# SludgePhD/Compeg

Measured on AMD Instinct MI355X. Metric: Mpixels/s decoded (4K 4:2:2 restart-interval baseline JPEG -> RGBA8 in HBM), higher is better.
Workload: dtype u32 bit-reader / i16 levels / f32 IDCT / u8 RGBA

## Files before the change

compeg_amd/csrc/desc.cpp:

```cpp
#include <cstdlib>
#include <cstring>
#include <vector>

#include "device_types.h"
#include "front.h"
#include "kernels_body.h"
#include "coop_body.h"

namespace compeg {

void fill_desc(const ImageData &img, ImageDesc &d);
void fill_coop(const ImageData &img, ImageDesc &d);
uint32_t max_wave_span(const uint32_t *starts, size_t nstarts, size_t nwords, uint32_t intervals, uint32_t group);
bool walk_state_shared(const ImageDesc &a, const ImageDesc &b);

void fill_desc(const ImageData &img, ImageDesc &d)
{
    d.walk = nullptr;
    const Metadata &md = img.metadata;
    memset(&d, 0, sizeof d);
    d.l2_entries = uint32_t(img.l2.size());
    d.fast_off = uint32_t((img.l2.size() + 1) & ~size_t(1));
    d.standard_entropy = (img.flags & COMPEG_PARSE_STANDARD_ENTROPY) ? 1u : 0u;
    d.total_intervals = md.total_restart_intervals;
    d.restart_interval = md.restart_interval;
    d.dus_per_mcu = md.dus_per_mcu;
    d.width_mcus = md.width_mcus;
    d.mcu_w = md.max_hsample * 8;
    d.mcu_h = md.max_vsample * 8;
    d.total_dus = img.total_dus();
    uint32_t k = 0;
    for (uint32_t c = 0; c < 3; c++) {
        const Component &cm = md.components[c];
        d.du_base[c] = k;
        for (uint32_t i = 0; i < cm.hsample * cm.vsample && k < kMaxDusPerMcu; i++, k++)
            d.comp_of_du |= c << (2 * k);
        d.dc_table[c] = cm.dchuff < 4 ? cm.dchuff : 4;
        d.ac_table[c] = cm.achuff < 4 ? cm.achuff : 4;
        d.fast_table[c] = (cm.achuff == 1 || cm.achuff == 3) ? cm.achuff >> 1 : 2;
        d.dc_quant[c] = md.qtables[cm.qtable & 3][0];
        d.hsample[c] = cm.hsample;
        d.vsample[c] = cm.vsample;
        for (int z = 0; z < kRetained; z++)
            d.quant[c][z] = float(md.qtables[cm.qtable & 3][z]);
        d.dc_fast_table[c] = (cm.dchuff == 0 || cm.dchuff == 2) ? cm.dchuff >> 1 : 2;
    }
    fill_coop(img, d);
    d.total_mcus = img.total_mcus();
    const bool is422 = md.dus_per_mcu == 4 && md.components[0].hsample == 2 && md.components[0].vsample == 1 &&
                       md.components[1].hsample == 1 && md.components[1].vsample == 1 &&
                       md.components[2].hsample == 1 && md.components[2].vsample == 1;
    bool ok = is422 && md.restart_interval != 0 && md.restart_interval <= (1u << 18) && d.zero_du_ok != 0;
    if (ok) {
        const uint32_t pair0 = (d.dc_fast_table[0] & 1u) | ((d.fast_table[0] & 1u) << 1);
        uint32_t pair1 = pair0;
        for (uint32_t c = 1; c < 3; c++) {
            const uint32_t pr = (d.dc_fast_table[c] & 1u) | ((d.fast_table[c] & 1u) << 1);
            if (pr != pair0 && pair1 == pair0)
                pair1 = pr;
            ok = ok && (pr == pair0 || pr == pair1);
        }
    }
    for (uint32_t c = 0; c < 3 && ok; c++) {
        ok = d.fast_table[c] < 2 && d.dc_fast_table[c] < 2;
        const uint16_t *l1 = img.l1 + size_t(d.dc_table[c] & 3u) * 256;
        for (uint32_t i = 0; i < 256 && ok; i++) {
            const uint16_t e = l1[i];
            if (!(e & 0x8000u)) {
                ok = (e & 0xffu) <= 15u;
                continue;
            }
            for (uint32_t j = 0; j < 256 && ok; j++) {
                const size_t idx = size_t(e & 0x7fffu) + j;
                ok = idx >= img.l2.size() || (img.l2[idx] & 0xffu) <= 15u;
            }
        }
    }
    d.mcu_ok = ok ? 1u : 0u;
}

void fill_coop(const ImageData &img, ImageDesc &d)
{
    const Metadata &md = img.metadata;
    d.coop_ok = 0;
    d.zero_du_ok = 0;
    memset(d.zero_du, 0, sizeof d.zero_du);
    const bool is422 = md.dus_per_mcu == 4 && md.components[0].hsample == 2 && md.components[0].vsample == 1 &&
                       md.components[1].hsample == 1 && md.components[1].vsample == 1 &&
                       md.components[2].hsample == 1 && md.components[2].vsample == 1;
    if (!is422 || md.restart_interval == 0)
        return;
    for (uint32_t c = 0; c < 3; c++)
        if (d.fast_table[c] >= 2 || d.dc_fast_table[c] >= 2)
            return;
    std::vector<uint16_t> l1(kL1Entries, 0);
    memcpy(l1.data(), img.l1, sizeof img.l1);
    const uint32_t none[4] = {0, 0, 0, 0};
    ImageDesc t = d;
    t.l2 = img.l2.data();
    t.words = nullptr;
    t.nwords = 0;
    HuffShared s{};
    s.l1 = l1.data();
    s.l2 = img.l2.empty() ? l1.data() : img.l2.data();
    s.l2_staged = uint32_t(img.l2.size());
    s.win = none;
    s.win_base = 0;
    s.win_len = 4;
    for (uint32_t c = 0; c < 3; c++) {
        PrefetchReader r;
        r.buf = 0;
        r.left = 0x80000000u;
        r.next_word = 0;
        r.pre = 0;
        ImageDesc tq = t;
        tq.standard_entropy = 0;
        const int32_t diff = decode_dc_diff(r, tq, s, d.dc_table[c] * 256u);
        if (diff < -32767 || diff > 32767)
            return;
        int16_t slot[kDuSlotBytes / 2] = {0};
        decode_ac_loop<false>(r, tq, s, d.ac_table[c] * 256u, slot);
        d.zero_du[c][0] = int16_t(diff);
        for (int z = 1; z < kRetained; z++)
            d.zero_du[c][z] = slot[z];
    }
    d.zero_du_ok = 1;
    d.coop_ok = md.restart_interval <= kCoopMaxRestart ? 1u : 0u;
}

bool walk_state_shared(const ImageDesc &a, const ImageDesc &b)
// ... 25 lines not shown
```

compeg_amd/csrc/device_types.h:

```cpp
#pragma once

#include <cstdint>

namespace compeg {

constexpr int kWave = 64;
constexpr int kRetained = 32;
constexpr int kMaxDusPerMcu = 6;
constexpr uint32_t kStripMcus = 32;

constexpr uint32_t kFastBits = 11;
constexpr uint32_t kFastEntries = 1u << kFastBits;
constexpr uint32_t kFastAdvEob = 64;
constexpr uint32_t kFastEscape = 15u;

constexpr uint32_t fast_entry(uint32_t ref, uint32_t zrl_advance)
{
    return (((ref & 0xffu) == 0u ? kFastAdvEob : ((ref & 0xffu) == 0xf0u ? zrl_advance : ((ref >> 4) & 15u) + 1u)) << 9) |
           ((((ref >> 8) & 31u) + (ref & 15u)) << 4) | (ref & 15u);
}

constexpr uint32_t kDcFastBits = 9;
constexpr uint32_t kDcFastEntries = 1u << kDcFastBits;

#ifndef CG_COOP_LEAN_MAX
#define CG_COOP_LEAN_MAX 40
#endif
constexpr uint32_t kCoopLeanMaxRestart = CG_COOP_LEAN_MAX;
struct CoopShape {
    uint32_t dpi, ipw, rounds, lpi, count, list_cap;
};
constexpr uint32_t kCoopSlotListCap = 20;
constexpr CoopShape coop_shape(uint32_t restart_interval, uint32_t waves)
{
    CoopShape sh{};
    sh.dpi = 4u * restart_interval;
    const uint32_t room = uint32_t(kWave) * (waves ? waves : 1u);
    sh.ipw = (sh.dpi != 0u && sh.dpi <= room) ? room / sh.dpi : 1u;
    sh.rounds = (sh.ipw * sh.dpi + uint32_t(kWave) - 1u) / uint32_t(kWave);
    const uint32_t share = (sh.dpi + (waves ? waves : 1u) - 1u) / (waves ? waves : 1u);
    const uint32_t fit = uint32_t(kWave) / sh.ipw;
    sh.lpi = share < fit ? (share ? share : 1u) : fit;
    sh.count = 1u + (sh.lpi - 1u) / 4u;
    const uint32_t per_sub = (sh.dpi + sh.count - 1u) / sh.count;
    sh.list_cap = (restart_interval > kCoopLeanMaxRestart && per_sub > 10u) ? ((per_sub + 15u) & ~3u) : kCoopSlotListCap;
    return sh;
}

constexpr int kDuSlotBytes = 80;

struct alignas(16) McuState {
    uint32_t info;
    int32_t pred[3];
};
constexpr uint32_t kMcuDead = 1u << 11;

struct ImageDesc {
    const uint32_t *words;
    const uint32_t *starts;
    const uint16_t *l1;
    const uint16_t *l2;
    uint32_t nwords;
    uint32_t nstarts;
    uint32_t l2_entries;
    uint32_t fast_off;
    uint32_t fast_table[3];
    uint32_t standard_entropy;
    uint32_t dc_fast_table[3];
    uint32_t coop_ok;
    uint32_t zero_du_ok;
    int16_t zero_du[3][kRetained];
    const uint32_t *walk;
    uint32_t total_intervals;
    uint32_t restart_interval;
    uint32_t dus_per_mcu;
    uint32_t width_mcus;
    uint32_t mcu_w, mcu_h;
    uint32_t total_dus;
    uint32_t comp_of_du;
    uint32_t dc_table[3];
    uint32_t ac_table[3];
    uint32_t dc_quant[3];
    uint32_t hsample[3], vsample[3];
    uint32_t du_base[3];
    float quant[3][kRetained];
    int16_t *ac;
    int32_t *dc;
    uint8_t *out;
    uint32_t out_w, out_h;
    uint32_t out_alloc_h;
    uint32_t out_pitch;
    uint32_t first_huff_block;
    uint32_t first_idct_block;
    uint32_t *mcu_word;
    McuState *mcu_state;
    uint32_t mcu_ok;
    uint32_t total_mcus;
};

struct HuffLdsPlan {
    uint32_t l2_entries_in_lds;
    uint32_t window_words;
    uint32_t waves_per_block;
    uint32_t total_bytes;
    uint32_t waves_that_fit;
    bool window_cut;
};

}
```

compeg_amd/csrc/kernels.hip:

```cpp
#include <hip/hip_runtime.h>

#include <algorithm>
#include <atomic>
#include <cstdio>
#include <cstdlib>

#include "kernels_body.h"
#include "coop_body.h"
#include "walk_body.h"
#include "kernels.h"
#include "lab.h"

namespace compeg {

struct DeviceLimits {
    uint32_t cus, lds_bytes;
};
static DeviceLimits device_limits()
{
    static std::atomic<uint64_t> known[64];
    int dev = 0;
    const bool indexed = hipGetDevice(&dev) == hipSuccess && dev >= 0 && dev < 64;
    if (indexed) {
        const uint64_t k = known[dev].load(std::memory_order_relaxed);
// ... 85 lines not shown
    if (wave_first >= d.total_intervals)
        return;

    HuffShared s;
    s.l1 = l1;
    s.l2 = l2;
    s.l2_staged = umin(l2_in_lds, d.fast_off + 2u * kFastEntries);
    s.win = win;
    s.win_base = win_base;
    s.win_len = win_len;
    s.du_slots = reinterpret_cast<uint8_t *>(win) + align16(window_words * 4u);
    entropy_wave_to_records<SAMPLES>(d, s, wave_first + lane, lane);
}

__global__ void __launch_bounds__(1024)
entropy_kernel(const ImageDesc *__restrict__ descs, uint32_t l2_in_lds, uint32_t window_words)
{
    entropy_kernel_body<false>(descs, l2_in_lds, window_words);
}

__global__ void __launch_bounds__(768)
entropy_samples_kernel(const ImageDesc *__restrict__ descs, uint32_t l2_in_lds, uint32_t window_words)
{
    entropy_kernel_body<true>(descs, l2_in_lds, window_words);
}

struct WindowAhead {
    const ImageDesc *descs;
    uint32_t image;
    bool any;
    uint32_t first;
    uint32_t window_words, lane;
    uint32_t *win;
    uint32_t raw_base, raw_end, base, len, sink;
    uint32_t *queue;
    uint32_t next, drawn, stride, units, waves_per_image, group;

    __device__ __forceinline__ void at(uint32_t du, uint32_t du_total)
    {
        if (queue) {
            if (du == 0u && lane == 0u)
                drawn = atomicAdd(queue, 1u);
            if (du == 1u) {
                next = (stride + uint32_t(__builtin_amdgcn_readfirstlane(int(drawn)))) * group;
                any = next < units;
                if (any) {
                    image = uint32_t(__builtin_amdgcn_readfirstlane(int(next / waves_per_image)));
                    first = uint32_t(__builtin_amdgcn_readfirstlane(int((next % waves_per_image) * kWave)));
                }
            }
        }
        if (!any)
            return;
        const ImageDesc *dn = descs + image;
        if (du == (queue ? 1u : 0u))
            wave_window_fetch(*dn, first, raw_base, raw_end);
        if (du_total >= 8u && du == (du_total >= 10u ? du_total - 8u : 2u)) {
            uint32_t b, l;
            wave_window_from(*dn, raw_base, raw_end, window_words, b, l);
            const uint32_t have = dn->nwords > b ? umin(l, dn->nwords - b) : 0u;
            auto *words = CG_GLOBAL(const uint32_t, dn->words);
            for (uint32_t v = lane * 32u; v < have; v += kWave * 32u)
                sink ^= words[b + v];
        }
        if (du_total >= 8u && du == (du_total >= 10u ? du_total - 5u : 5u))
            asm volatile("" ::"v"(sink));
    }

    __device__ __forceinline__ void decoded(uint32_t du, uint32_t du_total)
    {
        if (!any || du + 1u != du_total)
            return;
        const ImageDesc *dn = descs + image;
        uint32_t b, l;
        wave_window_from(*dn, raw_base, raw_end, window_words, b, l);
        base = uint32_t(__builtin_amdgcn_readfirstlane(int(b)));
        len = uint32_t(__builtin_amdgcn_readfirstlane(int(l)));
        stage_window(*dn, win, base, len, lane);
        __builtin_amdgcn_fence(__ATOMIC_RELEASE, "wavefront");
        __builtin_amdgcn_wave_barrier();
    }
};

template <class LAYOUT, uint32_t GROUP>
__device__ __forceinline__ void fused_kernel_body(const ImageDesc *__restrict__ descs, uint32_t l2_in_lds, uint32_t window_words,
                                                  uint32_t waves_per_image, uint32_t images, uint32_t *queue)
{
    constexpr uint32_t group = GROUP;
    extern __shared__ __attribute__((aligned(16))) uint8_t smem[];
    const uint32_t wave = uint32_t(__builtin_amdgcn_readfirstlane(int(threadIdx.x / kWave))), lane = threadIdx.x % kWave;
    uint32_t image = blockIdx.y, wave_first = (blockIdx.x * (blockDim.x / kWave) + wave) * kWave;
    bool has_work = true;
    if (waves_per_image) {
        const uint32_t flat = (blockIdx.x * (blockDim.x / kWave) + wave) * (queue ? group : 1u);
        image = flat / waves_per_image;
        wave_first = (flat % waves_per_image) * kWave;
        has_work = image < images;
        image = has_work ? image : images - 1u;
    }
    image = uint32_t(__builtin_amdgcn_readfirstlane(int(image)));
    wave_first = uint32_t(__builtin_amdgcn_readfirstlane(int(wave_first)));
    if (!waves_per_image && blockIdx.x * blockDim.x >= descs[image].total_intervals)
        return;
    has_work = has_work && wave_first < descs[image].total_intervals;

    uint16_t *l1 = reinterpret_cast<uint16_t *>(smem);
    uint16_t *l2 = l1 + kL1Entries;
    const uint32_t wave_area = align16(window_words * 4u) + kWave * kDuSlotBytes;
    uint8_t *wave_base = smem + align16((kL1Entries + l2_in_lds) * 2u);
    uint32_t *win = reinterpret_cast<uint32_t *>(wave_base + wave * wave_area);
    uint8_t *slots = reinterpret_cast<uint8_t *>(win) + align16(window_words * 4u);

    uint32_t win_base = 0, win_len = 0;
    if (has_work)
        wave_window(descs[image], wave_first, window_words, win_base, win_len);
    stage_luts_and_window(descs[image], l1, l2, l2_in_lds, threadIdx.x, blockDim.x, win, win_base, win_len, lane);
    __syncthreads();

    if (!has_work)
        return;

    const uint32_t stride = gridDim.x * (blockDim.x / kWave), units = waves_per_image * images;
    const uint32_t per_draw = waves_per_image && queue ? group : 1u;
    uint32_t flat = (blockIdx.x * (blockDim.x / kWave) + wave) * per_draw;
    for (;;) {
        const ImageDesc &d = descs[image];
        HuffShared s;
        s.l1 = l1;
        s.l2 = l2;
        s.l2_staged = umin(l2_in_lds, d.fast_off + 2u * kFastEntries);
        s.win = win;
        s.win_base = win_base;
        s.win_len = win_len;
        s.du_slots = slots;
        const bool draw = waves_per_image && queue && flat % per_draw == per_draw - 1u;
        flat += waves_per_image && queue ? 1u : stride;
        WindowAhead ahead;
        ahead.descs = descs;
        ahead.queue = draw ? queue : nullptr;
        ahead.stride = stride;
        ahead.units = units;
        ahead.waves_per_image = waves_per_image;
        ahead.group = per_draw;
        ahead.next = ahead.drawn = 0u;
        ahead.any = waves_per_image && !draw && flat < units;
        ahead.image = ahead.first = 0u;
        if (ahead.any) {
            ahead.image = uint32_t(__builtin_amdgcn_readfirstlane(int(flat / waves_per_image)));
            ahead.first = uint32_t(__builtin_amdgcn_readfirstlane(int((flat % waves_per_image) * kWave)));
        }
        ahead.window_words = window_words;
        ahead.lane = lane;
        ahead.win = win;
        ahead.sink = 0u;
        LAYOUT::decode(d, s, wave_first + lane, lane, ahead);
        if (!ahead.any)
            break;
        if (draw)
            flat = ahead.next;
        image = ahead.image;
        wave_first = ahead.first;
        win_base = ahead.base;
        win_len = ahead.len;
    }
}

constexpr uint32_t kMcuQueueGroup = 4;

template <bool WIDE, bool RECORDS = false>
struct Wave422 {
    template <class AHEAD>
    static __device__ __forceinline__ void decode(const ImageDesc &d, const HuffShared &s, uint32_t interval, uint32_t lane, AHEAD &ahead)
    {
        decode_wave_fused_422<AHEAD, WIDE, RECORDS>(d, s, interval, lane, ahead);
    }
};
#if !defined(CG_FUSED_BOUNDS) || !defined(COMPEG_LAB)
#define CG_FUSED_BOUNDS 768
#endif
__global__ void __launch_bounds__(CG_FUSED_BOUNDS)
decode_fused_422_kernel(const ImageDesc *__restrict__ descs, uint32_t l2_in_lds, uint32_t window_words,
                        uint32_t waves_per_image, uint32_t images, uint32_t *queue)
{
    fused_kernel_body<Wave422<false>, 1>(descs, l2_in_lds, window_words, waves_per_image, images, queue);
}
__global__ void __launch_bounds__(768)
decode_fused_422_mcu_kernel(const ImageDesc *__restrict__ descs, uint32_t l2_in_lds, uint32_t window_words,
                            uint32_t waves_per_image, uint32_t images, uint32_t *queue)
{
    fused_kernel_body<Wave422<true>, kMcuQueueGroup>(descs, l2_in_lds, window_words, waves_per_image, images, queue);
}
__global__ void __launch_bounds__(768)
decode_fused_422_mcu_rec_kernel(const ImageDesc *__restrict__ descs, uint32_t l2_in_lds, uint32_t window_words,
                                uint32_t waves_per_image, uint32_t images, uint32_t *queue)
{
    fused_kernel_body<Wave422<true, true>, kMcuQueueGroup>(descs, l2_in_lds, window_words, waves_per_image, images, queue);
}
template <int HS, int VS, int MC>
__device__ __forceinline__ void fused_layout_kernel_body(const ImageDesc *__restrict__ descs, uint32_t l2_in_lds, uint32_t window_words)
{
    extern __shared__ __attribute__((aligned(16))) uint8_t smem[];
    const ImageDesc &d = descs[blockIdx.y];
    const uint32_t first_interval = blockIdx.x * blockDim.x;
    if (first_interval >= d.total_intervals)
        return;
    uint16_t *l1 = reinterpret_cast<uint16_t *>(smem);
    uint16_t *l2 = l1 + kL1Entries;
    const uint32_t wave_area = align16(window_words * 4u) + kWave * kDuSlotBytes;
    uint8_t *wave_base = smem + align16((kL1Entries + l2_in_lds) * 2u);
    const uint32_t wave = uint32_t(__builtin_amdgcn_readfirstlane(int(threadIdx.x / kWave))), lane = threadIdx.x % kWave;
    uint32_t *win = reinterpret_cast<uint32_t *>(wave_base + wave * wave_area);
    const uint32_t wave_first = first_interval + wave * kWave;
    uint32_t win_base = 0, win_len = 0;
    if (wave_first < d.total_intervals)
        wave_window(d, wave_first, window_words, win_base, win_len);
    stage_luts_and_window(d, l1, l2, l2_in_lds, threadIdx.x, blockDim.x, win, win_base, win_len, lane);
    __syncthreads();
    if (wave_first >= d.total_intervals)
        return;
    HuffShared s;
    s.l1 = l1;
    s.l2 = l2;
    s.l2_staged = umin(l2_in_lds, d.fast_off + 2u * kFastEntries);
    s.win = win;
    s.win_base = win_base;
    s.win_len = win_len;
    s.du_slots = reinterpret_cast<uint8_t *>(win) + align16(window_words * 4u);
    decode_wave_fused_layout<HS, VS, MC>(d, s, wave_first + lane, lane);
}

__global__ void __launch_bounds__(512)
decode_fused_444_kernel(const ImageDesc *__restrict__ descs, uint32_t l2_in_lds, uint32_t window_words)
{
    fused_layout_kernel_body<1, 1, 2>(descs, l2_in_lds, window_words);
}
__global__ void __launch_bounds__(768)
decode_fused_444_single_kernel(const ImageDesc *__restrict__ descs, uint32_t l2_in_lds, uint32_t window_words)
{
    fused_layout_kernel_body<1, 1, 1>(descs, l2_in_lds, window_words);
}
__global__ void __launch_bounds__(512)
decode_fused_440_kernel(const ImageDesc *__restrict__ descs, uint32_t l2_in_lds, uint32_t window_words)
{
    fused_layout_kernel_body<1, 2, 2>(descs, l2_in_lds, window_words);
}
__global__ void __launch_bounds__(768)
decode_fused_440_single_kernel(const ImageDesc *__restrict__ descs, uint32_t l2_in_lds, uint32_t window_words)
{
    fused_layout_kernel_body<1, 2, 1>(descs, l2_in_lds, window_words);
}
__global__ void __launch_bounds__(512)
decode_fused_420_kernel(const ImageDesc *__restrict__ descs, uint32_t l2_in_lds, uint32_t window_words)
{
    fused_layout_kernel_body<2, 2, 1>(descs, l2_in_lds, window_words);
}

template <class WAVE>
__device__ __forceinline__ void fused_stream_kernel_body(const ImageDesc *__restrict__ descs, uint32_t l2_in_lds, uint32_t rows,
                                                         uint32_t stage_after, uint32_t stage_below, uint32_t waves_per_image, uint32_t images,
                                                         uint32_t *queue)
{
    extern __shared__ __attribute__((aligned(16))) uint8_t smem[];
    const uint32_t wave = uint32_t(__builtin_amdgcn_readfirstlane(int(threadIdx.x / kWave))), lane = threadIdx.x % kWave;
    uint32_t image = blockIdx.y, wave_first = (blockIdx.x * (blockDim.x / kWave) + wave) * kWave;
    bool has_work = true;
    if (waves_per_image) {
        const uint32_t flat = blockIdx.x * (blockDim.x / kWave) + wave;
// ... 981 lines not shown
```

compeg_amd/csrc/kernels_body.h:

```cpp
#pragma once

#include <cstdint>
#include <cstring>

#include "device_types.h"

#if defined(__HIPCC__)
#define CG_DEV __device__ __forceinline__
#else
#define CG_DEV static inline
#endif

#if defined(__HIP_DEVICE_COMPILE__)
#define CG_GLOBAL(T, p) (reinterpret_cast<__attribute__((address_space(1))) T *>(reinterpret_cast<uintptr_t>(p)))
#define CG_PIN_SCALAR(x) asm volatile("" : "+s"(x))
#else
#define CG_GLOBAL(T, p) (p)
#define CG_PIN_SCALAR(x) (void)(x)
#endif

#ifndef CG_IDCT_PACKED
#define CG_IDCT_PACKED 1
#endif
#ifndef CG_PRIO_IDCT
// ... 679 lines not shown
            uint32_t e2 = s.l2[idx < s.l2_staged ? idx : 0u];
            if (idx >= s.l2_staged)
                e2 = CG_GLOBAL(const uint16_t, d.l2)[idx < d.l2_entries ? idx : 0u];
            e = idx < d.l2_entries ? e2 : 0u;
        }
    }
    return e;
}

template <bool FAST>
CG_DEV uint32_t lut_resolve(const ImageDesc &d, const HuffShared &s, uint32_t e, uint32_t cur)
{
    if (e & 0x8000u) {
        const uint32_t idx = (e & 0x7fffu) + ((cur >> 16) & 0xffu);
        if (FAST) {
            e = idx < d.l2_entries ? s.l2[idx] : 0u;
        } else {
            uint32_t e2 = s.l2[idx < s.l2_staged ? idx : 0u];
            if (idx >= s.l2_staged)
                e2 = CG_GLOBAL(const uint16_t, d.l2)[idx < d.l2_entries ? idx : 0u];
            e = idx < d.l2_entries ? e2 : 0u;
        }
    }
    return e;
}

CG_DEV int32_t decode_dc_diff(PrefetchReader &r, const ImageDesc &d, const HuffShared &s,
                              uint32_t dc_off)
{
    if (d.standard_entropy)
        reader_refill<false>(r, d, s);
    const uint32_t e = lut_lookup<false>(d, s, dc_off, reader_cur(r));
    reader_consume(r, e >> 8);
    const uint32_t cat = e & 0xffu;
    const int32_t raw = int32_t(reader_peek(r, cat));
    reader_consume(r, cat);
    return huff_extend(raw, cat);
}

template <bool FAST>
CG_DEV void decode_ac_loop(PrefetchReader &r, const ImageDesc &d, const HuffShared &s,
                           uint32_t ac_off, int16_t *slot16, uint32_t pos0 = 1u)
{
    uint32_t pos = pos0;
    reader_refill<FAST>(r, d, s);
    uint32_t e = lut_lookup<FAST>(d, s, ac_off, reader_cur(r));
    bool done;
    do {
        const uint32_t len = e >> 8, sym = e & 0xffu, nb = sym & 15u;
        const uint32_t t = reader_cur(r) << (len & 31u);
        reader_consume(r, len + nb);

        const bool need = r.left < 32u;
        const uint64_t buf_n = merge_word(r.buf, r.pre, r.left, need);
        const uint32_t nw_n = r.next_word + (need ? 1u : 0u);
        const uint32_t cur_n = uint32_t(buf_n >> 32);
        const uint32_t e1_n = s.l1[ac_off + (cur_n >> 24)];
        const uint32_t pre_n = fetch_word_pf<FAST>(d, s, nw_n);

        const uint32_t raw = (t >> 1) >> (31u - nb);
        const uint32_t neg = ~uint32_t(int32_t(t) >> 31);
        const uint32_t val = raw + (neg & ((0xffffffffu << nb) + 1u));
        const uint32_t p = pos + (sym >> 4);
        slot16[p < uint32_t(kRetained) ? p : uint32_t(kRetained)] = int16_t(val);
        pos = sym == 0u ? 64u : p + ((sym == 0xf0u && !d.standard_entropy) ? 2u : 1u);
        done = pos >= 64u;

        r.buf = done ? r.buf : buf_n;
        r.left += (need && !done) ? 32u : 0u;
        r.next_word = done ? r.next_word : nw_n;
        r.pre = done ? r.pre : pre_n;
        e = lut_resolve<FAST>(d, s, e1_n, cur_n);
    } while (!done);
}

struct EntropyState {
    PrefetchReader r;
    const uint32_t *wptr;
    uint32_t ref_left;
    bool fast;
    int32_t pred0, pred1, pred2;
    const uint32_t *wlimit;
    bool resume;
};

#if defined(CG_EMUL_STATS)
struct EmulStats {
    unsigned long fast_dus, exact_dus, left_window, left_underflow, dc_cut, escapes;
    unsigned long symbols, lane_symbols, wave_steps, wave_step_symbols;
};
inline EmulStats g_emul_stats{};
#define CG_COUNT(field) (++g_emul_stats.field)
#else
#define CG_COUNT(field) ((void)0)
#endif

#if defined(__HIP_DEVICE_COMPILE__)
#define CG_LDS(T, p) (reinterpret_cast<__attribute__((address_space(3))) T *>(reinterpret_cast<uintptr_t>(p)))
#else
#define CG_LDS(T, p) (p)
#endif

CG_DEV uint32_t lds_read_u16_early(const uint16_t *p)
{
#if defined(__HIP_DEVICE_COMPILE__)
    uint32_t v;
    asm volatile("ds_read_u16 %0, %1" : "=v"(v) : "v"(uint32_t(reinterpret_cast<uintptr_t>(p))) : "memory");
    return v;
#else
    return *p;
#endif
}

CG_DEV uint32_t lds_read_u32_early(const uint32_t *p)
{
#if defined(__HIP_DEVICE_COMPILE__)
    uint32_t v;
    asm volatile("ds_read_b32 %0, %1" : "=v"(v) : "v"(uint32_t(reinterpret_cast<uintptr_t>(p))) : "memory");
    return v;
#else
    return *p;
#endif
}

CG_DEV void lds_reads_done(uint32_t &a, uint32_t &b)
{
#if defined(__HIP_DEVICE_COMPILE__)
    asm volatile("s_waitcnt lgkmcnt(0)" : "+v"(a), "+v"(b)::"memory");
#else
    (void)a;
    (void)b;
#endif
}

CG_DEV void lds_reads_done3(uint32_t &a, uint32_t &b, uint32_t &c)
{
#if defined(__HIP_DEVICE_COMPILE__)
    asm volatile("s_waitcnt lgkmcnt(0)" : "+v"(a), "+v"(b), "+v"(c)::"memory");
#else
    (void)a;
    (void)b;
    (void)c;
#endif
}

CG_DEV bool fast_tables_usable(const ImageDesc &d, const HuffShared &s)
{
    return d.fast_table[0] < 2u && d.fast_table[1] < 2u && d.fast_table[2] < 2u &&
           s.l2_staged >= d.fast_off + 2u * kFastEntries;
}

CG_DEV void entropy_init(EntropyState &e, const ImageDesc &d, const HuffShared &s, uint32_t interval)
{
    reader_init(e.r, d, s, interval < d.nstarts ? CG_GLOBAL(const uint32_t, d.starts)[interval] : 0u);
    reader_refill<false>(e.r, d, s);
    e.pred0 = e.pred1 = e.pred2 = 0;
    e.ref_left = 32u;
    const uint32_t rel = e.r.next_word - s.win_base;
    e.fast = fast_tables_usable(d, s) && rel < s.win_len;
    e.wptr = s.win + (e.fast ? rel : 0u);
}

CG_DEV uint32_t stream_word_index(const EntropyState &e, const HuffShared &s, uint32_t lane)
{
    return e.r.next_word + uint32_t(e.wptr - (s.win + lane)) / uint32_t(kWave);
}

template <bool STREAM = false>
CG_DEV void leave_fast_mode(EntropyState &e, const ImageDesc &d, const HuffShared &s, uint32_t lane = 0u)
{
    PrefetchReader &r = e.r;
    if (d.standard_entropy)
        e.ref_left = r.left;
    const uint32_t ahead = (r.left - e.ref_left) >> 5;
    if (STREAM) {
        r.next_word = stream_word_index(e, s, lane) - ahead;
        r.pre = fetch_word_pf<false>(d, s, r.next_word);
    } else {
        r.next_word = s.win_base + uint32_t(e.wptr - s.win) - ahead;
        if (ahead)
            r.pre = fetch_word_pf<false>(d, s, r.next_word);
    }
    r.buf &= ~uint64_t(0) << (64u - e.ref_left);
    r.left = e.ref_left;
    e.fast = false;
}

CG_DEV void stream_leave_inside(EntropyState &e, const ImageDesc &d, const HuffShared &s, uint32_t lane)
{
    PrefetchReader &r = e.r;
    r.next_word = stream_word_index(e, s, lane);
    r.pre = fetch_word_pf<false>(d, s, r.next_word);
    e.fast = false;
    e.resume = true;
}

template <bool STREAM = false>
CG_DEV void fast_refill(EntropyState &e)
{
    PrefetchReader &r = e.r;
    const uint32_t t = r.left - 32u;
    const uint32_t f = t >> 31;
    const uint32_t w = (STREAM ? bswap32(r.pre) : r.pre) & uint32_t(int32_t(t) >> 31);
    r.buf |= (uint64_t(w) << 32) >> (r.left & 63u);
    r.left += f << 5;
    e.wptr += STREAM ? f * uint32_t(kWave) : f;
#if CG_EXP == 12
    r.pre = uint32_t(reinterpret_cast<uintptr_t>(e.wptr)) * 2654435761u;
#else
    r.pre = lds_read_u32_early(e.wptr);
#endif
}

CG_DEV int32_t signed_field(uint32_t cur, uint32_t tot, uint32_t nb)
{
#if defined(__HIP_DEVICE_COMPILE__)
    return __builtin_amdgcn_sbfe(int32_t(cur), 32u - tot, nb);
#else
    return nb ? int32_t(cur << (tot - nb)) >> (32u - nb) : 0;
#endif
}

CG_DEV bool fast_dc(EntropyState &e, const ImageDesc &d, const HuffShared &s, uint32_t dc_off, int32_t &diff)
{
    PrefetchReader &r = e.r;
    if (d.standard_entropy)
        e.ref_left = r.left;
    const uint32_t seen = e.ref_left < 32u ? e.ref_left : 32u;
    if (e.ref_left < 32u)
        CG_COUNT(dc_cut);
    const uint32_t cur = reader_cur(r) & ~uint32_t(uint64_t(0xffffffffu) >> seen);
    const uint32_t ent = lut_lookup<true>(d, s, dc_off, cur);
    const uint32_t len = ent >> 8, cat = ent & 0xffu, n = len + cat;
    if (n > e.ref_left || cat > 16u)
        return false;
    const int32_t raw = int32_t(((cur << (len & 31u)) >> 1) >> (31u - cat));
    diff = huff_extend(raw, cat);
    r.buf <<= n;
    r.left -= n;
    return true;
}

#if defined(CG_AC_STAMPS) && defined(__HIPCC__)
__device__ unsigned long long g_ac_stamps[4];
#endif
#if defined(CG_AC_STAMPS) && defined(__HIP_DEVICE_COMPILE__)
#define CG_AC_STAMP(x) x
#else
#define CG_AC_STAMP(x)
#endif

template <bool STREAM = false>
CG_DEV uint32_t fast_ac(EntropyState &e, const ImageDesc &d, const HuffShared &s, uint32_t ac_off,
                        uint32_t fast_base, int16_t *slot16)
{
    CG_AC_STAMP(const uint64_t ts0 = __builtin_readcyclecounter(); uint64_t tw = 0; uint32_t its = 0;)
    PrefetchReader &r = e.r;
    const uint16_t *tab = s.l2 + fast_base;
    if (STREAM && e.wptr >= e.wlimit)
        return 0u;
    fast_refill<STREAM>(e);
    uint32_t ent = lds_read_u16_early(tab + (reader_cur(r) >> (32u - kFastBits)));
    uint32_t at = 0u, tot = 0u;
    int16_t *pend_at = slot16 + kRetained;
    int16_t pend_val = 0;
    while (at < 63u && (!STREAM || e.wptr < e.wlimit)) {
        CG_AC_STAMP(const uint64_t tw0 = __builtin_readcyclecounter();)
        lds_reads_done(ent, r.pre);
        CG_AC_STAMP(tw += __builtin_readcyclecounter() - tw0; its++;)
#if CG_EXP != 12
        *pend_at = pend_val;
#endif
#if CG_EXP != 7
        if (__builtin_expect(ent == kFastEscape, 0))
#else
        if (false)
#endif
        {
            CG_COUNT(escapes);
            ent = fast_entry(lut_lookup<true>(d, s, ac_off, reader_cur(r)), d.standard_entropy ? 16u : 17u);
        }
#if CG_EXP >= 10 && CG_EXP <= 12
        ent = (5u << 9) | (5u << 4) | 2u;
#endif
        const uint32_t nb = ent & 15u, adv = ent >> 9;
        tot = (ent >> 4) & 31u;
        const uint32_t cur = reader_cur(r);
        r.buf <<= tot;
        r.left -= tot;
        fast_refill<STREAM>(e);
#if CG_EXP == 11 || CG_EXP == 12
        ent = reader_cur(r) >> 30;
#else
        ent = lds_read_u16_early(tab + (reader_cur(r) >> (32u - kFastBits)));
#endif
        const int32_t sx = signed_field(cur, tot, nb);
        const uint32_t val = uint32_t(sx) + (((0xffffffffu << nb) ^ uint32_t(sx >> 31)) + 1u);
        at += adv;
        CG_COUNT(symbols);
        CG_COUNT(lane_symbols);
        pend_at = slot16 + umin(at, uint32_t(kRetained));
        pend_val = int16_t(val);
    }
    lds_reads_done(ent, r.pre);
    *pend_at = pend_val;
    CG_AC_STAMP(if ((threadIdx.x & 63u) == 0u) {
        atomicAdd(&g_ac_stamps[0], __builtin_readcyclecounter() - ts0);
        atomicAdd(&g_ac_stamps[1], tw);
        atomicAdd(&g_ac_stamps[2], its);
        atomicAdd(&g_ac_stamps[3], 1ull);
    })
    e.ref_left = 32u + ((r.left + tot) & 31u) - tot;
    return at;
}

template <bool STREAM = false>
CG_DEV int32_t entropy_data_unit(EntropyState &e, const ImageDesc &d, const HuffShared &s, uint32_t comp,
                                 int16_t *slot16, uint32_t lane = 0u)
{
    const uint32_t dc_off = d.dc_table[comp] * 256u, ac_off = d.ac_table[comp] * 256u;
    int32_t diff = 0;
    bool decoded = false;
    if (!STREAM && e.fast) {
        const uint32_t rel = uint32_t(e.wptr - s.win);
        if (s.win_len - rel < kDuWordSlack) {
            CG_COUNT(left_window);
            leave_fast_mode(e, d, s);
        }
    }
    if (STREAM && e.fast) {
        if (fast_dc(e, d, s, dc_off, diff)) {
            const uint32_t at = fast_ac<true>(e, d, s, ac_off, d.fast_off + d.fast_table[comp] * kFastEntries, slot16);
            CG_COUNT(fast_dus);
            if (at < 63u) {
                CG_COUNT(left_window);
                stream_leave_inside(e, d, s, lane);
                decode_ac_loop<false>(e.r, d, s, ac_off, slot16, at + 1u);
            }
            decoded = true;
        } else {
            CG_COUNT(left_underflow);
            leave_fast_mode<true>(e, d, s, lane);
        }
    } else if (e.fast) {
        if (fast_dc(e, d, s, dc_off, diff)) {
#if CG_EXP == 3
            {
                const EntropyState saved = e;
                fast_ac(e, d, s, ac_off, d.fast_off + d.fast_table[comp] * kFastEntries, slot16);
                e = saved;
            }
#endif
            fast_ac(e, d, s, ac_off, d.fast_off + d.fast_table[comp] * kFastEntries, slot16);
            decoded = true;
            CG_COUNT(fast_dus);
        } else {
            CG_COUNT(left_underflow);
            leave_fast_mode(e, d, s);
        }
    }
    if (!decoded) {
        CG_COUNT(exact_dus);
        diff = decode_dc_diff(e.r, d, s, dc_off);
        decode_ac_loop<false>(e.r, d, s, ac_off, slot16);
    }
    const int32_t p0 = e.pred0, p1 = e.pred1, p2 = e.pred2;
    const int32_t p = int32_t(uint32_t(comp == 0u ? p0 : (comp == 1u ? p1 : p2)) + uint32_t(diff));
    e.pred0 = comp == 0u ? p : p0;
    e.pred1 = comp == 1u ? p : p1;
    e.pred2 = comp == 2u ? p : p2;
    return int32_t(uint32_t(p) * d.dc_quant[comp]);
}


constexpr int kPxSlotWords = 17;

CG_DEV uint32_t ycbcr_to_rgba(uint32_t y_, uint32_t cb_, uint32_t cr_)
{
    const int32_t y = int32_t(y_), cb = int32_t(cb_) - 128, cr = int32_t(cr_) - 128;
    int32_t r = y + ((45 * cr) >> 5);
    int32_t g = y - ((11 * cb + 23 * cr) >> 5);
    int32_t b = y + ((113 * cb) >> 6);
    r = r < 0 ? 0 : (r > 255 ? 255 : r);
    g = g < 0 ? 0 : (g > 255 ? 255 : g);
    b = b < 0 ? 0 : (b > 255 ? 255 : b);
    return uint32_t(r) | uint32_t(g) << 8 | uint32_t(b) << 16 | 0xff000000u;
}

CG_DEV void composite_422(const ImageDesc &d, const uint32_t *px_slots, uint32_t first_mcu,
                          uint32_t total_mcus, uint32_t j)
{
    const uint32_t m = j >> 2, quarter = j & 3u;
    const uint32_t mcu = first_mcu + m;
    if (mcu >= total_mcus)
        return;
    const uint32_t mx = mcu % d.width_mcus, my = mcu / d.width_mcus;
    const uint32_t x0 = mx * 16u + quarter * 4u;
    if (x0 >= d.out_w)
        return;
    const uint32_t *ydu = px_slots + (m * 4u + (quarter >> 1)) * kPxSlotWords;
    const uint32_t *cbdu = px_slots + (m * 4u + 2u) * kPxSlotWords;
    const uint32_t *crdu = px_slots + (m * 4u + 3u) * kPxSlotWords;
    const uint32_t cshift = (quarter & 1u) * 16u;
#pragma unroll
    for (uint32_t row = 0; row < 8; row++) {
        const uint32_t y = my * 8u + row;
        if (y >= d.out_h)
            break;
        const uint32_t yw = ydu[row * 2u + (quarter & 1u)];
        const uint32_t cbw = cbdu[row * 2u + (quarter >> 1)] >> cshift;
        const uint32_t crw = crdu[row * 2u + (quarter >> 1)] >> cshift;
        Vec4u o;
        o.x = ycbcr_to_rgba(yw & 0xffu, cbw & 0xffu, crw & 0xffu);
        o.y = ycbcr_to_rgba((yw >> 8) & 0xffu, cbw & 0xffu, crw & 0xffu);
        o.z = ycbcr_to_rgba((yw >> 16) & 0xffu, (cbw >> 8) & 0xffu, (crw >> 8) & 0xffu);
        o.w = ycbcr_to_rgba(yw >> 24, (cbw >> 8) & 0xffu, (crw >> 8) & 0xffu);
        uint8_t *p = d.out + size_t(y) * d.out_pitch + size_t(x0) * 4u;
        if (x0 + 3u < d.out_w && (d.out_pitch & 15u) == 0u) {
            store_pixels<true>(p, o);
        } else {
            auto *q = CG_GLOBAL(uint32_t, reinterpret_cast<uint32_t *>(p));
            q[0] = o.x;
            if (x0 + 1u < d.out_w)
                q[1] = o.y;
            if (x0 + 2u < d.out_w)
                q[2] = o.z;
            if (x0 + 3u < d.out_w)
                q[3] = o.w;
        }
    }
}


CG_DEV uint32_t ycbcr_to_rgba(uint32_t y_, uint32_t cb_, uint32_t cr_);

CG_DEV Vec4u rgba_quad(uint32_t yw, uint32_t cb2, uint32_t cr2)
{
    Vec4u o;
#if defined(__HIP_DEVICE_COMPILE__)
    typedef short s2 __attribute__((ext_vector_type(2)));
// ... 567 lines not shown
        }
        pixel_next_mcu(t, d);
        return;
    }
    const uint64_t addr = reinterpret_cast<uint64_t>(g.base);
    const uint32_t lo = uint32_t(addr), hi = uint32_t(addr >> 32), wh = g.whole ? 1u : 0u;
    uint8_t *slot = wave_slots + lane * kDuSlotBytes;
    if (WIDE) {
        uint8_t *from[4] = {
            reinterpret_cast<uint8_t *>(uint64_t(wave_lane<0>(hi, lane)) << 32 | wave_lane<0>(lo, lane)),
            reinterpret_cast<uint8_t *>(uint64_t(wave_lane<1>(hi, lane)) << 32 | wave_lane<1>(lo, lane)),
            reinterpret_cast<uint8_t *>(uint64_t(wave_lane<2>(hi, lane)) << 32 | wave_lane<2>(lo, lane)),
            reinterpret_cast<uint8_t *>(uint64_t(wave_lane<3>(hi, lane)) << 32 | wave_lane<3>(lo, lane)),
        };
        const uint32_t mask = wave_lane<0>(wh, lane) | wave_lane<1>(wh, lane) << 1 | wave_lane<2>(wh, lane) << 2 | wave_lane<3>(wh, lane) << 3;
        if (__builtin_amdgcn_ballot_w64(mask != 0xfu) == 0u) {
#pragma unroll
            for (uint32_t row = 0; row < 8; row++) {
                composite_row_to_slot(t.px, row, slot);
                composite_row_from_wave(d, wave_slots, lane, row, from, 0xfu);
                __builtin_amdgcn_sched_barrier(0);
            }
        } else {
#pragma unroll
            for (uint32_t row = 0; row < 8; row++) {
                composite_row_to_slot(t.px, row, slot);
                composite_row_from_wave(d, wave_slots, lane, row, from, mask);
                __builtin_amdgcn_sched_barrier(0);
            }
        }
        zero_slot(slot);
        if (t.active && !g.whole)
            composite_edge_mcu(d, t.px, t.mx, t.my);
        pixel_next_mcu(t, d);
        return;
    }
    uint8_t *bases[4] = {
        reinterpret_cast<uint8_t *>(uint64_t(quad_lane<0>(hi)) << 32 | quad_lane<0>(lo)),
        reinterpret_cast<uint8_t *>(uint64_t(quad_lane<1>(hi)) << 32 | quad_lane<1>(lo)),
        reinterpret_cast<uint8_t *>(uint64_t(quad_lane<2>(hi)) << 32 | quad_lane<2>(lo)),
        reinterpret_cast<uint8_t *>(uint64_t(quad_lane<3>(hi)) << 32 | quad_lane<3>(lo)),
    };
    const uint32_t whole_mask = quad_lane<0>(wh) | quad_lane<1>(wh) << 1 | quad_lane<2>(wh) << 2 | quad_lane<3>(wh) << 3;
#if CG_EXP == 15
    if (__builtin_amdgcn_ballot_w64(whole_mask != 0xfu) == 0u) {
        uint8_t *left[4] = {bases[0] - 64, bases[1] - 64, bases[2] - 64, bases[3] - 64};
#pragma unroll
        for (uint32_t row = 0; row < 8; row++) {
            composite_row_to_slot(t.px, row, slot);
            if (t.mx & 1u) {
                composite_row_from_quad(d, wave_slots, lane, row, left, 0xfu);
                composite_row_from_quad(d, wave_slots, lane, row, bases, 0xfu);
            }
            __builtin_amdgcn_sched_barrier(0);
        }
    } else
#endif
    if (__builtin_amdgcn_ballot_w64(whole_mask != 0xfu) == 0u) {
#pragma unroll
        for (uint32_t row = 0; row < 8; row++) {
            composite_row_to_slot(t.px, row, slot);
            composite_row_from_quad(d, wave_slots, lane, row, bases, 0xfu);
            __builtin_amdgcn_sched_barrier(0);
        }
    } else {
#pragma unroll
        for (uint32_t row = 0; row < 8; row++) {
            composite_row_to_slot(t.px, row, slot);
            composite_row_from_quad(d, wave_slots, lane, row, bases, whole_mask);
            __builtin_amdgcn_sched_barrier(0);
        }
    }
    zero_slot(slot);
    if (t.active && !g.whole)
        composite_edge_mcu(d, t.px, t.mx, t.my);
    pixel_next_mcu(t, d);
}

struct NothingAhead {
    CG_DEV void at(uint32_t, uint32_t) {}
    CG_DEV void decoded(uint32_t, uint32_t) {}
};

template <class AHEAD, bool WIDE = false, bool RECORDS = false>
CG_DEV void decode_wave_fused_422(const ImageDesc &d, const HuffShared &s, uint32_t interval, uint32_t lane, AHEAD &ahead)
{
    const bool active = interval < d.total_intervals;
    interval = active ? interval : d.total_intervals - 1u;
    uint8_t *slot = s.du_slots + lane * kDuSlotBytes;
    int16_t *slot16 = reinterpret_cast<int16_t *>(slot);
    zero_slot(slot);

    EntropyState e;
    PixelState t;
    if (RECORDS)
        entropy_init_from_record(e, d, s, interval);
    else
        entropy_init(e, d, s, interval);
    pixel_init(t, d, interval, active);
    __builtin_amdgcn_s_setprio(CG_PRIO_ENTROPY);

#if defined(CG_STAMPS) && defined(__HIP_DEVICE_COMPILE__)
#define CG_STAMP(acc) do { const uint64_t now_ = __builtin_readcyclecounter(); acc += now_ - tprev; tprev = now_; } while (0)
    uint64_t tprev = __builtin_readcyclecounter(), t_dc = 0, t_ac = 0, t_idct = 0, t_comp = 0;
#else
#define CG_STAMP(acc) do { } while (0)
#endif
    const uint32_t du_total = d.restart_interval * 4u;
#pragma unroll 1
    for (uint32_t du = 0; du < du_total; du++) {
        const uint32_t k = du & 3u;
        const uint32_t comp = k < 2u ? 0u : k - 1u;
        ahead.at(du, du_total);
        const int32_t dc = entropy_data_unit(e, d, s, comp, slot16);
        CG_STAMP(t_ac);
        ahead.decoded(du, du_total);
        __builtin_amdgcn_s_setprio(CG_PRIO_IDCT);
        pixel_transform(t, d, comp, k, slot, dc);
        CG_STAMP(t_idct);
        if (k == 3u) {
            __builtin_amdgcn_s_setprio(CG_PRIO_COMPOSITE);
            composite_mcus_422<true, WIDE>(t, d, s.du_slots, lane);
            CG_STAMP(t_comp);
        }
        __builtin_amdgcn_s_setprio(CG_PRIO_ENTROPY);
    }
#if defined(CG_STAMPS) && defined(__HIP_DEVICE_COMPILE__)
    if (lane == 0 && d.dc) {
        uint64_t *o = reinterpret_cast<uint64_t *>(d.dc) + size_t(interval / 64u) * 4u;
        o[0] = t_dc;
        o[1] = t_ac;
        o[2] = t_idct;
        o[3] = t_comp;
    }
#endif
}

CG_DEV void decode_wave_fused_422(const ImageDesc &d, const HuffShared &s, uint32_t interval, uint32_t lane)
{
    NothingAhead none;
    decode_wave_fused_422(d, s, interval, lane, none);
}

CG_DEV void decode_wave_fused_422_stream(const ImageDesc &d, const HuffShared &s, uint32_t nrows, uint32_t stage_after, uint32_t stage_below,
                                         uint32_t interval, uint32_t lane)
{
    const bool active = interval < d.total_intervals;
    interval = active ? interval : d.total_intervals - 1u;
    uint8_t *slot = s.du_slots + lane * kDuSlotBytes;
    int16_t *slot16 = reinterpret_cast<int16_t *>(slot);
    zero_slot(slot);

    EntropyState e;
    PixelState t;
    stream_lane_init(e, d, s, nrows, interval, lane);
    pixel_init(t, d, interval, active);
    stream_rows_landed();
    __builtin_amdgcn_s_setprio(CG_PRIO_ENTROPY);

    const uint32_t du_total = d.restart_interval * 4u;
#pragma unroll 1
    for (uint32_t du = 0; du < du_total; du++) {
        const uint32_t k = du & 3u;
        const uint32_t comp = k < 2u ? 0u : k - 1u;
        const int32_t dc = entropy_data_unit<true>(e, d, s, comp, slot16, lane);
        bool stage = ((stage_after | 8u) >> k & 1u) != 0u && du + 1u < du_total;
        if (stage)
            stage = wave_any(stream_wants_rows(e, d, s, lane, stage_below));
        if (stage)
            stream_restage(e, d, s, nrows, lane);
        __builtin_amdgcn_s_setprio(CG_PRIO_IDCT);
        pixel_transform(t, d, comp, k, slot, dc);
        if (stage)
            stream_rows_landed();
        if (k == 3u) {
            __builtin_amdgcn_s_setprio(CG_PRIO_COMPOSITE);
            composite_mcus_422<true>(t, d, s.du_slots, lane);
        }
        __builtin_amdgcn_s_setprio(CG_PRIO_ENTROPY);
    }
}

#endif

template <int HS, int VS, int MC>
struct LayoutPixels {
    static constexpr int kDus = HS * VS + 2;
    uint32_t px[MC * kDus][16];
    uint32_t mx, my;
    bool active;
};

template <int HS, int VS, int MC>
CG_DEV Vec4u layout_pixels4(const LayoutPixels<HS, VS, MC> &t, int row, int g)
{
    constexpr int kDus = HS * VS + 2;
    const int m = g / (2 * HS), gg = g % (2 * HS), o = m * kDus;
// ... 332 lines not shown
```

Before: 755,100.

## Decode two AC Huffman symbols per lookup using pair tables in LDS

Builds 10-bit pair lookup tables in LDS from the existing 11-bit fast AC tables, where each 32-bit entry encodes up to two consecutive Huffman symbols. A new fast_ac_pairs loop consumes both symbols per iteration, with deferred coefficient stores, aiming to halve the serial lookup-dependency chain in AC decoding. It adds a table construction pass with two block barriers per kernel launch, and it has more complex per-step bit extraction. A host-side validity check gates second-symbol packing.

```diff
diff --git a/compeg_amd/csrc/desc.cpp b/compeg_amd/csrc/desc.cpp
--- a/compeg_amd/csrc/desc.cpp
+++ b/compeg_amd/csrc/desc.cpp
@@ -13,6 +13,31 @@
 void fill_coop(const ImageData &img, ImageDesc &d);
 uint32_t max_wave_span(const uint32_t *starts, size_t nstarts, size_t nwords, uint32_t intervals, uint32_t group);
 bool walk_state_shared(const ImageDesc &a, const ImageDesc &b);
+
+static uint32_t pair_tables_ok(const std::vector<uint16_t> &fast)
+{
+    uint32_t ok = 0;
+    for (uint32_t t = 0; t < 2 && fast.size() >= 2u * kFastEntries; t++) {
+        const uint16_t *tab = fast.data() + size_t(t) * kFastEntries;
+        bool good = true;
+        for (uint32_t x = 0; x < kFastEntries && good;) {
+            const uint32_t e = tab[x];
+            if (e == kFastEscape) {
+                x++;
+                continue;
+            }
+            const uint32_t len = ((e >> 4) & 31u) - (e & 15u);
+            good = len >= 1u && len <= kFastBits;
+            const uint32_t block = good ? 1u << (kFastBits - len) : 1u;
+            good = good && (x & (block - 1u)) == 0u;
+            for (uint32_t y = x; y < x + block && good; y++)
+                good = tab[y] == e;
+            x += block;
+        }
+        ok |= (good ? 1u : 0u) << t;
+    }
+    return ok;
+}
 
 void fill_desc(const ImageData &img, ImageDesc &d)
 {
@@ -46,6 +71,7 @@
         d.dc_fast_table[c] = (cm.dchuff == 0 || cm.dchuff == 2) ? cm.dchuff >> 1 : 2;
     }
     fill_coop(img, d);
+    d.pair_ok = pair_tables_ok(img.ac_fast);
     d.total_mcus = img.total_mcus();
     const bool is422 = md.dus_per_mcu == 4 && md.components[0].hsample == 2 && md.components[0].vsample == 1 &&
                        md.components[1].hsample == 1 && md.components[1].vsample == 1 &&
diff --git a/compeg_amd/csrc/device_types.h b/compeg_amd/csrc/device_types.h
--- a/compeg_amd/csrc/device_types.h
+++ b/compeg_amd/csrc/device_types.h
@@ -19,6 +19,9 @@
     return (((ref & 0xffu) == 0u ? kFastAdvEob : ((ref & 0xffu) == 0xf0u ? zrl_advance : ((ref >> 4) & 15u) + 1u)) << 9) |
            ((((ref >> 8) & 31u) + (ref & 15u)) << 4) | (ref & 15u);
 }
+
+constexpr uint32_t kPairBits = 10;
+constexpr uint32_t kPairEntries = 1u << kPairBits;
 
 constexpr uint32_t kDcFastBits = 9;
 constexpr uint32_t kDcFastEntries = 1u << kDcFastBits;
@@ -96,6 +99,7 @@
     McuState *mcu_state;
     uint32_t mcu_ok;
     uint32_t total_mcus;
+    uint32_t pair_ok;
 };
 
 struct HuffLdsPlan {
diff --git a/compeg_amd/csrc/kernels.hip b/compeg_amd/csrc/kernels.hip
--- a/compeg_amd/csrc/kernels.hip
+++ b/compeg_amd/csrc/kernels.hip
@@ -191,6 +191,26 @@
     }
 };
 
+constexpr uint32_t kPairsPerThread = 2u * kPairEntries / uint32_t(kWave);
+__device__ __forceinline__ void make_pair_tables(uint16_t *direct, uint32_t pair_ok, uint32_t tid, uint32_t nthreads)
+{
+    uint32_t v[kPairsPerThread];
+#pragma unroll
+    for (uint32_t j = 0; j < kPairsPerThread; j++) {
+        const uint32_t i = tid + j * nthreads, t = i / kPairEntries;
+        v[j] = i < 2u * kPairEntries ? pair_entry(direct + t * kFastEntries, i % kPairEntries, (pair_ok >> t) & 1u) : 0u;
+    }
+    __syncthreads();
+    uint32_t *pairs = reinterpret_cast<uint32_t *>(direct);
+#pragma unroll
+    for (uint32_t j = 0; j < kPairsPerThread; j++) {
+        const uint32_t i = tid + j * nthreads;
+        if (i < 2u * kPairEntries)
+            pairs[i] = v[j];
+    }
+    __syncthreads();
+}
+
 template <class LAYOUT, uint32_t GROUP>
 __device__ __forceinline__ void fused_kernel_body(const ImageDesc *__restrict__ descs, uint32_t l2_in_lds, uint32_t window_words,
                                                   uint32_t waves_per_image, uint32_t images, uint32_t *queue)
@@ -225,6 +245,8 @@
         wave_window(descs[image], wave_first, window_words, win_base, win_len);
     stage_luts_and_window(descs[image], l1, l2, l2_in_lds, threadIdx.x, blockDim.x, win, win_base, win_len, lane);
     __syncthreads();
+    if (LAYOUT::kPairs && descs[image].fast_off + 2u * kFastEntries <= l2_in_lds)
+        make_pair_tables(l2 + descs[image].fast_off, descs[image].pair_ok, threadIdx.x, blockDim.x);
 
     if (!has_work)
         return;
@@ -276,12 +298,13 @@
 
 constexpr uint32_t kMcuQueueGroup = 4;
 
-template <bool WIDE, bool RECORDS = false>
+template <bool WIDE, bool RECORDS = false, bool PAIRS = false>
 struct Wave422 {
+    static constexpr bool kPairs = PAIRS;
     template <class AHEAD>
     static __device__ __forceinline__ void decode(const ImageDesc &d, const HuffShared &s, uint32_t interval, uint32_t lane, AHEAD &ahead)
     {
-        decode_wave_fused_422<AHEAD, WIDE, RECORDS>(d, s, interval, lane, ahead);
+        decode_wave_fused_422<AHEAD, WIDE, RECORDS, PAIRS>(d, s, interval, lane, ahead);
     }
 };
 #if !defined(CG_FUSED_BOUNDS) || !defined(COMPEG_LAB)
@@ -291,7 +314,7 @@
 decode_fused_422_kernel(const ImageDesc *__restrict__ descs, uint32_t l2_in_lds, uint32_t window_words,
                         uint32_t waves_per_image, uint32_t images, uint32_t *queue)
 {
-    fused_kernel_body<Wave422<false>, 1>(descs, l2_in_lds, window_words, waves_per_image, images, queue);
+    fused_kernel_body<Wave422<false, false, true>, 1>(descs, l2_in_lds, window_words, waves_per_image, images, queue);
 }
 __global__ void __launch_bounds__(768)
 decode_fused_422_mcu_kernel(const ImageDesc *__restrict__ descs, uint32_t l2_in_lds, uint32_t window_words,
diff --git a/compeg_amd/csrc/kernels_body.h b/compeg_amd/csrc/kernels_body.h
--- a/compeg_amd/csrc/kernels_body.h
+++ b/compeg_amd/csrc/kernels_body.h
@@ -785,12 +785,16 @@
     int32_t pred0, pred1, pred2;
     const uint32_t *wlimit;
     bool resume;
+#if defined(CG_EMUL_STATS)
+    bool pair_end;
+#endif
 };
 
 #if defined(CG_EMUL_STATS)
 struct EmulStats {
     unsigned long fast_dus, exact_dus, left_window, left_underflow, dc_cut, escapes;
     unsigned long symbols, lane_symbols, wave_steps, wave_step_symbols;
+    unsigned long pair_steps, pairs, pair_du_ends, underflow_after_pair;
 };
 inline EmulStats g_emul_stats{};
 #define CG_COUNT(field) (++g_emul_stats.field)
@@ -862,6 +866,9 @@
     const uint32_t rel = e.r.next_word - s.win_base;
     e.fast = fast_tables_usable(d, s) && rel < s.win_len;
     e.wptr = s.win + (e.fast ? rel : 0u);
+#if defined(CG_EMUL_STATS)
+    e.pair_end = false;
+#endif
 }
 
 CG_DEV uint32_t stream_word_index(const EntropyState &e, const HuffShared &s, uint32_t lane)
@@ -1017,7 +1024,82 @@
     return at;
 }
 
-template <bool STREAM = false>
+CG_DEV uint32_t pair_entry(const uint16_t *direct, uint32_t idx, bool second)
+{
+    const uint32_t prefix = idx << (kFastBits - kPairBits);
+    const uint32_t e1 = direct[prefix];
+    const uint32_t tot1 = (e1 >> 4) & 31u;
+    if (e1 == kFastEscape || tot1 - (e1 & 15u) > kPairBits)
+        return kFastEscape;
+    uint32_t hi = tot1 << 4;
+    if (second && (e1 >> 9) != kFastAdvEob && tot1 < kPairBits) {
+        const uint32_t e2 = direct[(prefix << tot1) & (kFastEntries - 1u)];
+        const uint32_t tot2 = (e2 >> 4) & 31u;
+        if (e2 != kFastEscape && tot2 - (e2 & 15u) <= kPairBits - tot1 && tot1 + tot2 <= 31u)
+            hi = (e2 & ~0x1f0u) | ((tot1 + tot2) << 4);
+    }
+    return e1 | hi << 16;
+}
+
+CG_DEV uint32_t fast_ac_pairs(EntropyState &e, const ImageDesc &d, const HuffShared &s, uint32_t ac_off,
+                              const uint32_t *tab, int16_t *slot16)
+{
+    PrefetchReader &r = e.r;
+    fast_refill(e);
+    uint32_t ent = lds_read_u32_early(tab + (reader_cur(r) >> (32u - kPairBits)));
+    uint32_t at = 0u, tot = 0u, tot1 = 0u;
+    int16_t *pend_at1 = slot16 + kRetained, *pend_at2 = slot16 + kRetained;
+    int16_t pend_val1 = 0, pend_val2 = 0;
+    while (at < 63u) {
+        lds_reads_done(ent, r.pre);
+        *pend_at2 = pend_val2;
+        *pend_at1 = pend_val1;
+        if (__builtin_expect(ent == kFastEscape, 0)) {
+            CG_COUNT(escapes);
+            ent = fast_entry(lut_lookup<true>(d, s, ac_off, reader_cur(r)), d.standard_entropy ? 16u : 17u);
+            ent |= (ent & 0x1f0u) << 16;
+        }
+        const uint32_t nb1 = ent & 15u, adv1 = (ent >> 9) & 127u, nb2 = (ent >> 16) & 15u, adv2 = ent >> 25;
+        const uint32_t tot12 = (ent >> 20) & 31u;
+        tot1 = (ent >> 4) & 31u;
+        const uint32_t at1 = at + adv1;
+        tot = at1 < 63u ? tot12 : tot1;
+        const uint32_t cur = reader_cur(r);
+        r.buf <<= tot;
+        r.left -= tot;
+        fast_refill(e);
+        ent = lds_read_u32_early(tab + (reader_cur(r) >> (32u - kPairBits)));
+        const int32_t sx1 = signed_field(cur, tot1, nb1), sx2 = signed_field(cur, tot12, nb2);
+        const uint32_t val1 = uint32_t(sx1) + (((0xffffffffu << nb1) ^ uint32_t(sx1 >> 31)) + 1u);
+        const uint32_t val2 = uint32_t(sx2) + (((0xffffffffu << nb2) ^ uint32_t(sx2 >> 31)) + 1u);
+        at = at1 + adv2;
+#if defined(CG_EMUL_STATS)
+        CG_COUNT(pair_steps);
+        CG_COUNT(symbols);
+        CG_COUNT(lane_symbols);
+        if (tot != tot1) {
+            CG_COUNT(pairs);
+            CG_COUNT(symbols);
+            CG_COUNT(lane_symbols);
+            if (at >= 63u)
+                CG_COUNT(pair_du_ends);
+        }
+        e.pair_end = tot != tot1;
+#endif
+        pend_at1 = slot16 + umin(at1, uint32_t(kRetained));
+        pend_at2 = slot16 + umin(at, uint32_t(kRetained));
+        pend_val1 = int16_t(val1);
+        pend_val2 = int16_t(val2);
+    }
+    lds_reads_done(ent, r.pre);
+    *pend_at2 = pend_val2;
+    *pend_at1 = pend_val1;
+    const uint32_t last = tot != tot1 ? tot - tot1 : tot1;
+    e.ref_left = 32u + ((r.left + last) & 31u) - last;
+    return at;
+}
+
+template <bool STREAM = false, bool PAIRS = false>
 CG_DEV int32_t entropy_data_unit(EntropyState &e, const ImageDesc &d, const HuffShared &s, uint32_t comp,
                                  int16_t *slot16, uint32_t lane = 0u)
 {
@@ -1054,11 +1136,19 @@
                 e = saved;
             }
 #endif
-            fast_ac(e, d, s, ac_off, d.fast_off + d.fast_table[comp] * kFastEntries, slot16);
+            if (PAIRS)
+                fast_ac_pairs(e, d, s, ac_off, reinterpret_cast<const uint32_t *>(s.l2 + d.fast_off) + d.fast_table[comp] * kPairEntries,
+                              slot16);
+            else
+                fast_ac(e, d, s, ac_off, d.fast_off + d.fast_table[comp] * kFastEntries, slot16);
             decoded = true;
             CG_COUNT(fast_dus);
         } else {
             CG_COUNT(left_underflow);
+#if defined(CG_EMUL_STATS)
+            if (PAIRS && e.pair_end)
+                CG_COUNT(underflow_after_pair);
+#endif
             leave_fast_mode(e, d, s);
         }
     }
@@ -1792,7 +1882,7 @@
     CG_DEV void decoded(uint32_t, uint32_t) {}
 };
 
-template <class AHEAD, bool WIDE = false, bool RECORDS = false>
+template <class AHEAD, bool WIDE = false, bool RECORDS = false, bool PAIRS = false>
 CG_DEV void decode_wave_fused_422(const ImageDesc &d, const HuffShared &s, uint32_t interval, uint32_t lane, AHEAD &ahead)
 {
     const bool active = interval < d.total_intervals;
@@ -1822,7 +1912,7 @@
         const uint32_t k = du & 3u;
         const uint32_t comp = k < 2u ? 0u : k - 1u;
         ahead.at(du, du_total);
-        const int32_t dc = entropy_data_unit(e, d, s, comp, slot16);
+        const int32_t dc = entropy_data_unit<false, PAIRS>(e, d, s, comp, slot16);
         CG_STAMP(t_ac);
         ahead.decoded(du, du_total);
         __builtin_amdgcn_s_setprio(CG_PRIO_IDCT);
```

Result: no change. 757,100 (median of 6 runs) (+0.3%).
